# Lapis-Hong/wide_deep

Measured on NVIDIA H100. Metric: CTR examples/sec (train step), higher is better.
Workload: dtype bf16x3 (fp32 operands split into bf16 hi+lo, 3 tensor-core products, fp32 accumulate; 2^-16)

## Files before the change

### include/wd_b200.h

```cpp
#ifndef WD_B200_H_
#define WD_B200_H_

#include <stddef.h>
#include <stdint.h>

#ifdef __cplusplus
extern "C" {
#endif

#define WD_API_VERSION 3

enum { WD_OK = 0, WD_EINVAL = -1, WD_ENODEVICE = -2, WD_ECUDA = -3, WD_ENOMEM = -4, WD_EUNSUPPORTED = -5, WD_ESTATE = -6 };

enum { WD_COL_HASH = 0, WD_COL_VOCAB = 1, WD_COL_IDENTITY = 2, WD_COL_BUCKET = 3, WD_COL_CROSS = 4 };
enum { WD_NORM_NONE = 0, WD_NORM_MINMAX = 1, WD_NORM_STANDARD = 2, WD_NORM_LOG = 3 };
enum { WD_KEY_FIELD = 0, WD_KEY_COLUMN = 1 };
enum { WD_OPT_SGD = 0, WD_OPT_ADAGRAD = 1, WD_OPT_FTRL = 2,
       WD_OPT_ADAM = 3     ,
       WD_OPT_RMSPROP = 4   };
enum { WD_ACT_RELU = 0, WD_ACT_RELU6, WD_ACT_SIGMOID, WD_ACT_TANH, WD_ACT_LEAKY_RELU, WD_ACT_ELU, WD_ACT_SELU,
       WD_ACT_SOFTPLUS, WD_ACT_SOFTSIGN,
       WD_ACT_CRELU    };
enum { WD_MODE_SIMPLE = 0, WD_MODE_FIRST_DENSE, WD_MODE_LAST_DENSE, WD_MODE_DENSE, WD_MODE_RESNET };
enum { WD_GEMM_AUTO = 0, WD_GEMM_FFMA = 1, WD_GEMM_TC3X = 2 ,
// ... 134 lines not shown

int wd_eval_reset(WdModel *m);
int wd_eval_accumulate(WdModel *m, const WdBatch *batch);
int wd_eval_finish(WdModel *m, double *out10);
int wd_eval_accumulate_slot(WdModel *m, int slot);

int wd_fingerprint64_device(const uint8_t *bytes, const int64_t *offsets, int64_t n, uint64_t *out);
uint64_t wd_fingerprint64(const uint8_t *bytes, size_t n);
uint64_t wd_fingerprint_cat64(uint64_t a, uint64_t b);

int wd_debug_column_ids(WdModel *m, int32_t *offsets_out, int64_t offsets_cap, int64_t *ids_out, int64_t ids_cap, int64_t *nnz_out);
int wd_debug_slot(WdModel *m, int slot, int32_t *batch_out, int64_t *nnz_out, int32_t *parts_out, int32_t *offsets_out,
                  uint64_t *keys_out, float *dense_out, float *label_out, float *weight_out);
int wd_debug_deep_input(WdModel *m, float *out, int64_t cap);
int wd_debug_hidden(WdModel *m, int tower, int layer, float *out, int64_t cap);
int64_t wd_launch_count(WdModel *m);
int64_t wd_gemm_fallback_count(WdModel *m);
int wd_graph_stats(WdModel *m, int64_t *out, int32_t n);
int wd_last_timings(WdModel *m, float *ms_out, int cap);
const char *wd_timing_name(WdModel *m, int i);
int wd_set_profile(WdModel *m, int enable);
void *wd_stream(WdModel *m);
int wd_debug_gemm_probe(unsigned long long *out);
void *wd_stream_sparse(WdModel *m, int which);
int wd_sync(WdModel *m);

#define WD_SUMMARY_BUCKETS 1551
enum { WD_SEG_DEEP_INPUT = 0, WD_SEG_HIDDEN = 1, WD_SEG_TOWER_LOGITS = 2, WD_SEG_WIDE_LOGIT = 3 };
int wd_summary_limits(double *out, int32_t cap);
int wd_summary_segments(WdModel *m, int32_t *kind, int32_t *tower, int32_t *layer, int32_t cap);
int wd_summary_arm(WdModel *m);
int wd_summary_read(WdModel *m, int64_t *counts, int64_t *ints, double *reals, int32_t n_segments);

typedef struct WdTsvSpec {
    int32_t n_columns;
    const int32_t *col_role;
    const int32_t *col_target;
    int32_t n_cat_fields, n_dense_fields;
    int32_t multivalue;
    int32_t tf_compat_pad;
    float pos_weight, neg_weight;
    int32_t use_weight;
    int32_t has_label;
} WdTsvSpec;
int64_t wd_tsv_parse(const WdTsvSpec *spec, const char *text, int64_t text_len, int32_t n_lines,
                     int32_t *offsets_out, uint64_t *keys_out, int64_t keys_cap,
// ... 20 lines not shown
```

### wide_deep_b200/_native.py

```python
import ctypes
import os

_HERE = os.path.dirname(os.path.abspath(__file__))
SO_PATH = os.path.join(_HERE, "libwd_b200.so")
_lib = None

OK, EINVAL, ENODEVICE, ECUDA, ENOMEM, EUNSUPPORTED, ESTATE = 0, -1, -2, -3, -4, -5, -6


class NativeError(RuntimeError):
    def __init__(self, code, msg):
        super().__init__("libwd_b200 error %d: %s" % (code, msg))
        self.code = code


class BatchC(ctypes.Structure):
    _fields_ = [("batch_size", ctypes.c_int32), ("cat_offsets", ctypes.c_void_p), ("cat_keys", ctypes.c_void_p),
                ("nnz", ctypes.c_int64), ("dense", ctypes.c_void_p), ("label", ctypes.c_void_p), ("weight", ctypes.c_void_p)]


class TsvSpecC(ctypes.Structure):
    _fields_ = [("n_columns", ctypes.c_int32), ("col_role", ctypes.c_void_p), ("col_target", ctypes.c_void_p),
                ("n_cat_fields", ctypes.c_int32), ("n_dense_fields", ctypes.c_int32), ("multivalue", ctypes.c_int32),
                ("tf_compat_pad", ctypes.c_int32), ("pos_weight", ctypes.c_float), ("neg_weight", ctypes.c_float),
# ... 44 lines not shown
    "wd_shard_eval_accumulate_phase": (ctypes.c_int, [_vp, _i32]),
    "wd_shard_eval_finish": (ctypes.c_int, [_vp, _vp]),
    "wd_eval_reset": (ctypes.c_int, [_vp]),
    "wd_eval_accumulate": (ctypes.c_int, [_vp, _vp]),
    "wd_eval_finish": (ctypes.c_int, [_vp, _vp]),
    "wd_eval_accumulate_slot": (ctypes.c_int, [_vp, ctypes.c_int]),
    "wd_fingerprint64_device": (ctypes.c_int, [_vp, _vp, _i64, _vp]),
    "wd_fingerprint64": (_u64, [ctypes.c_char_p, ctypes.c_size_t]),
    "wd_fingerprint_cat64": (_u64, [_u64, _u64]),
    "wd_debug_column_ids": (ctypes.c_int, [_vp, _vp, _i64, _vp, _i64, ctypes.POINTER(_i64)]),
    "wd_debug_slot": (ctypes.c_int, [_vp, ctypes.c_int, ctypes.POINTER(_i32), ctypes.POINTER(_i64), ctypes.POINTER(_i32), _vp, _vp, _vp,
                                     _vp, _vp]),
    "wd_debug_deep_input": (ctypes.c_int, [_vp, _vp, _i64]),
    "wd_debug_hidden": (ctypes.c_int, [_vp, ctypes.c_int, ctypes.c_int, _vp, _i64]),
    "wd_launch_count": (_i64, [_vp]),
    "wd_gemm_fallback_count": (_i64, [_vp]),
    "wd_graph_stats": (ctypes.c_int, [_vp, ctypes.POINTER(_i64), _i32]),
    "wd_last_timings": (ctypes.c_int, [_vp, _vp, ctypes.c_int]),
    "wd_timing_name": (ctypes.c_char_p, [_vp, ctypes.c_int]),
    "wd_batch_upload_slot": (ctypes.c_int, [_vp, ctypes.c_int, _vp]),
    "wd_batch_prefetch_slot": (ctypes.c_int, [_vp, ctypes.c_int, _vp]),
    "wd_last_loss": (ctypes.c_int, [_vp, _vp]),
    "wd_debug_gemm_probe": (ctypes.c_int, [_vp]),
    "wd_train_step_slot": (ctypes.c_int, [_vp, ctypes.c_int, ctypes.POINTER(ctypes.c_float)]),
    "wd_set_profile": (ctypes.c_int, [_vp, ctypes.c_int]),
    "wd_stream": (_vp, [_vp]),
    "wd_stream_sparse": (_vp, [_vp, ctypes.c_int]),
    "wd_sync": (ctypes.c_int, [_vp]),
    "wd_host_alloc": (ctypes.c_int, [ctypes.c_size_t, ctypes.POINTER(_vp)]),
    "wd_host_free": (ctypes.c_int, [_vp]),
    "wd_tsv_parse": (_i64, [_vp, ctypes.c_char_p, _i64, _i32, _vp, _vp, _i64, _vp, _vp, _vp, _i32]),
    "wd_tsv_index_lines": (_i64, [_vp, _i64, _vp, _vp, _i64]),
    "wd_tsv_parse_lines": (_i64, [_vp, _vp, _vp, _vp, _vp, _i32, _vp, _vp, _i64, _vp, _vp, _vp, _i32]),
    "wd_tsv_gather_lines": (_i64, [_vp, _vp, _vp, _vp, _i32, _vp, _i64, _vp, _i32]),
    "wd_tsv_parse_slot": (ctypes.c_int, [_vp, ctypes.c_int, _vp, _vp, _i64, _vp, _i32]),
    "wd_tsv_parse_stats": (ctypes.c_int, [_vp, ctypes.POINTER(_i64), _i32, _i32]),
    "wd_summary_limits": (ctypes.c_int, [_vp, _i32]),
    "wd_summary_segments": (ctypes.c_int, [_vp, _vp, _vp, _vp, _i32]),
    "wd_summary_arm": (ctypes.c_int, [_vp]),
    "wd_summary_read": (ctypes.c_int, [_vp, _vp, _vp, _vp, _i32]),
}


def lib():
    global _lib
    if _lib is None:
# ... 15 lines not shown
```

### wide_deep_b200/csrc/gemm.cuh

```cuda
#pragma once
#include <cuda.h>
#include <cuda_bf16.h>

#include "common.cuh"

namespace wd {

__device__ __forceinline__ float act_fwd(int kind, float z) {
    switch (kind) {
        case WD_ACT_RELU: return fmaxf(z, 0.f);
        case WD_ACT_RELU6: return fminf(fmaxf(z, 0.f), 6.f);
        case WD_ACT_SIGMOID: return 1.f / (1.f + expf(-z));
        case WD_ACT_TANH: return tanhf(z);
        case WD_ACT_LEAKY_RELU: return z > 0.f ? z : 0.2f * z;
        case WD_ACT_ELU: return z > 0.f ? z : expm1f(z);
        case WD_ACT_SELU: return 1.0507009873554805f * (z > 0.f ? z : 1.6732632423543772f * expm1f(z));
        case WD_ACT_SOFTPLUS: return fmaxf(z, 0.f) + log1pf(expf(-fabsf(z)));
        case WD_ACT_SOFTSIGN: return z / (1.f + fabsf(z));
    }
    return z;
}
__device__ __forceinline__ float act_bwd(int kind, float a) {
    switch (kind) {
        case WD_ACT_RELU: return a > 0.f ? 1.f : 0.f;
// ... 18 lines not shown
    const __nv_bfloat16* lo[kMaxSegs];
};
struct GemmB {
    const float* ptr; int ld;
    const float *tf32_hi, *tf32_lo;
    const __nv_bfloat16 *hi, *lo;
};
enum { EPI_FWD = 0, EPI_STORE = 1, EPI_WGRAD = 2 };
struct Epi {
    float* C; int ldc;
    int accumulate;
    float* A_out; float* H_out; int ldh;
    float* HT; int ldt;
    const float *bias, *gamma, *beta;
    int n_logical, act, bn;
    int m_valid;
    int64_t split_stride;
    __nv_bfloat16 *Hs_hi, *Hs_lo;
    uint64_t reserved[5];
};

int tc_gemm(WdModel* m, int mode, const GemmA& A, const GemmB& B, int M, int N, const Epi& ep, int splits, int ksplit_len);
int tc_gemm_bf16(WdModel* m, int mode, const GemmA& A, const GemmB& B, int M, int N, const Epi& ep, int splits, int ksplit_len);
int make_tensor_map(CUtensorMap* map, CUtensorMapDataType dtype, const void* ptr, int rows, int cols, int ld, int box_rows);

struct DropArgs { float rate; unsigned long long seed; const unsigned int* step; int layer_id; unsigned int row0; };
__device__ __forceinline__ unsigned long long splitmix64_dev(unsigned long long x) {
    x += 0x9E3779B97F4A7C15ULL;
    x = (x ^ (x >> 30)) * 0xBF58476D1CE4E5B9ULL;
    x = (x ^ (x >> 27)) * 0x94D049BB133111EBULL;
    return x ^ (x >> 31);
}
__device__ __forceinline__ unsigned long long drop_key(const DropArgs& d) {
    return splitmix64_dev(d.seed ^ ((unsigned long long)(*d.step) * 0x9E3779B97F4A7C15ULL) ^ ((unsigned long long)d.layer_id << 48));
}
__device__ __forceinline__ float drop_mult(unsigned long long key, unsigned int m, unsigned int n, float rate, float inv_keep) {
    const unsigned long long r = splitmix64_dev(key ^ ((unsigned long long)m * 65536ULL + n));
    const float u = (float)(unsigned int)(r >> 40) * (1.f / 16777216.f);
    return u >= rate ? inv_keep : 0.f;
}

__device__ __forceinline__ float bn_out(float a, const float* __restrict__ gamma, const float* __restrict__ beta, int n, int bn) {
    return bn ? fmaf(a, gamma[n] * 0.99950037468777f, beta[n]) : a;
}

__device__ __forceinline__ void split_bf16(float x, __nv_bfloat16& hi, __nv_bfloat16& lo) {
    hi = __float2bfloat16_rn(x);
// ... 18 lines not shown
```

### wide_deep_b200/csrc/gemm_bf16.cu

```cuda
#include <cuda.h>
#include <stdlib.h>

#include <algorithm>
#include <type_traits>

#include "common.cuh"
#include "gemm.cuh"
#include "wgmma_ptx.cuh"

namespace wd {

namespace {

constexpr int QBM = 128;
constexpr int QBN = 128;
constexpr int QNST = 3;
constexpr int QBK = 64;
constexpr int Q_THREADS = 384;

struct QMaps {
    CUtensorMap a_hi[kMaxSegs], a_lo[kMaxSegs];
    CUtensorMap b_hi, b_lo;
};
struct QSegs { int n; int k[kMaxSegs]; int koff[kMaxSegs]; };

__device__ unsigned long long g_probe[32 * 8];
__device__ __forceinline__ unsigned long long gtime() { unsigned long long t; asm volatile("mov.u64 %0, %globaltimer;" : "=l"(t)); return t; }
#define PROBE(i) do { if (probe >= 0 && blockIdx.x == 0 && (threadIdx.x & 127) == 0) g_probe[probe * 8 + (i)] = gtime(); } while (0)

template <int MODE>
__global__ void __launch_bounds__(Q_THREADS, 1) tc_gemm_bf16_kernel(const __grid_constant__ QMaps maps, const QSegs segs, int M, int N, int ktot,
                                                                   int ksplit_len, int nsplit, Epi ep, int probe) {
    extern __shared__ uint8_t smem_raw[];
    uint8_t* base = reinterpret_cast<uint8_t*>((reinterpret_cast<uintptr_t>(smem_raw) + 1023) & ~uintptr_t(1023));
    constexpr bool A_MN = MODE == EPI_WGRAD;
    constexpr bool B_MN = MODE == EPI_FWD || MODE == EPI_WGRAD;
    constexpr int A_BYTES = QBM * 128, B_BYTES = QBN * 128;
    constexpr int STAGE_BYTES = 2 * (A_BYTES + B_BYTES);
    auto a_hi = [&](int s) { return base + s * STAGE_BYTES; };
    auto a_lo = [&](int s) { return base + s * STAGE_BYTES + A_BYTES; };
    auto b_hi = [&](int s) { return base + s * STAGE_BYTES + 2 * A_BYTES; };
    auto b_lo = [&](int s) { return base + s * STAGE_BYTES + 2 * A_BYTES + B_BYTES; };
    uint64_t* bars = reinterpret_cast<uint64_t*>(base + QNST * STAGE_BYTES);
    uint64_t* full = bars; uint64_t* empty = bars + QNST;
    float* epi_vec = reinterpret_cast<float*>(base + QNST * STAGE_BYTES + 64);

    const int warp = threadIdx.x >> 5, lane = threadIdx.x & 31, wg = threadIdx.x >> 7;
    const int tiles_n = (N + QBN - 1) / QBN, tiles_m = (M + QBM - 1) / QBM;
    const int ntiles = tiles_n * tiles_m * nsplit;
    int nkb_all = 0;
    for (int s = 0; s < segs.n; ++s) nkb_all += (segs.k[s] + QBK - 1) / QBK;
    auto tile_range = [&](int tile, int& m0, int& n0, int& z, int& kbeg, int& nkb) {
        z = tile / (tiles_n * tiles_m);
        int r = tile % (tiles_n * tiles_m);
        m0 = (r / tiles_n) * QBM;
        n0 = (r % tiles_n) * QBN;
        kbeg = 0;
        nkb = nkb_all;
        if (MODE == EPI_WGRAD) {
            kbeg = z * ksplit_len;
            int kend = min(ktot, kbeg + ksplit_len);
            nkb = kend > kbeg ? (kend - kbeg + QBK - 1) / QBK : 0;
        }
    };

    if (threadIdx.x == 0) {
        for (int s = 0; s < QNST; ++s) { mbar_init(&full[s], 1); mbar_init(&empty[s], 8); }
        asm volatile("fence.mbarrier_init.release.cluster;" ::: "memory");
    }
    __syncthreads();

    if (wg == 0) {
        reg_dealloc<40>();
        PROBE(0);
        if (warp == 0 && lane == 0) {
            int g = 0;
            for (int tile = blockIdx.x; tile < ntiles; tile += gridDim.x) {
                int m0, n0, z, kbeg, nkb;
                tile_range(tile, m0, n0, z, kbeg, nkb);
                int seg = 0, kin = 0;
                for (int kb = 0; kb < nkb; ++kb, ++g) {
                    const int s = g % QNST, it = g / QNST;
                    if (it > 0) mbar_wait(&empty[s], (it - 1) & 1);
                    int ka, kbcoord;
                    if (MODE == EPI_WGRAD) { ka = kbeg + kb * QBK; kbcoord = ka; }
                    else {
                        if (kin >= segs.k[seg]) { ++seg; kin = 0; }
                        ka = kin; kbcoord = segs.koff[seg] + kin;
                        kin += QBK;
                    }
                    mbar_expect_tx(&full[s], 2 * (A_BYTES + B_BYTES));
                    if (!A_MN) {
                        tma_load_2d(a_hi(s), &maps.a_hi[seg], &full[s], ka, m0);
                        tma_load_2d(a_lo(s), &maps.a_lo[seg], &full[s], ka, m0);
                    } else {
#pragma unroll
                        for (int i = 0; i < QBM / 64; ++i) {
                            tma_load_2d(a_hi(s) + i * 8192, &maps.a_hi[seg], &full[s], m0 + 64 * i, ka);
                            tma_load_2d(a_lo(s) + i * 8192, &maps.a_lo[seg], &full[s], m0 + 64 * i, ka);
                        }
                    }
                    if (!B_MN) {
                        tma_load_2d(b_hi(s), &maps.b_hi, &full[s], kbcoord, n0);
                        tma_load_2d(b_lo(s), &maps.b_lo, &full[s], kbcoord, n0);
                    } else {
#pragma unroll
                        for (int i = 0; i < QBN / 64; ++i) {
                            tma_load_2d(b_hi(s) + i * 8192, &maps.b_hi, &full[s], n0 + 64 * i, kbcoord);
                            tma_load_2d(b_lo(s) + i * 8192, &maps.b_lo, &full[s], n0 + 64 * i, kbcoord);
                        }
                    }
                }
            }
        }
    } else {
        reg_alloc<232>();
        const int cw = wg - 1, cwarp = warp - 4;
        constexpr uint32_t a_step = A_MN ? 2048u : 32u, b_step = B_MN ? 2048u : 32u;
        constexpr int TA = A_MN ? 1 : 0, TB = B_MN ? 1 : 0;
        float d[QBN / 2];
        int g = 0, use = 0;
        for (int tile = blockIdx.x; tile < ntiles; tile += gridDim.x) {
            int m0, n0, z, kbeg, nkb;
            tile_range(tile, m0, n0, z, kbeg, nkb);
            if (nkb == 0) {
#pragma unroll
                for (int i = 0; i < QBN / 2; ++i) d[i] = 0.f;
            }
            const int ct = threadIdx.x - 128;
            float pre[2] = {0.f, 0.f};
            if (MODE == EPI_FWD) {
#pragma unroll
                for (int i = 0; i < 2; ++i) {
                    const int v = ct + 256 * i, c = n0 + (v & 127);
                    const bool in = c < ep.n_logical;
                    if (v < 128) pre[i] = in ? __ldg(ep.bias + c) : 0.f;
                    else if (v < 256) pre[i] = (in && ep.bn) ? __ldg(ep.gamma + c) * 0.99950037468777f : 1.f;
                    else if (v < 384) pre[i] = (in && ep.bn) ? __ldg(ep.beta + c) : 0.f;
                }
            }
            int prev = -1;
            for (int kb = 0; kb < nkb; ++kb, ++g) {
                const int s = g % QNST, it = g / QNST;
                mbar_wait(&full[s], it & 1);
                if (g == 0) PROBE(1);
                const uint32_t sa_hi = smem_u32(a_hi(s)) + cw * 8192, sa_lo = smem_u32(a_lo(s)) + cw * 8192;
                const uint32_t sb_hi = smem_u32(b_hi(s)), sb_lo = smem_u32(b_lo(s));
                wgmma_fence();
#pragma unroll
                for (int k = 0; k < QBK / 16; ++k) {
                    const uint64_t da_hi = A_MN ? make_desc_mn(sa_hi + k * a_step) : make_desc(sa_hi + k * a_step);
                    const uint64_t da_lo = A_MN ? make_desc_mn(sa_lo + k * a_step) : make_desc(sa_lo + k * a_step);
                    const uint64_t db_hi = B_MN ? make_desc_mn(sb_hi + k * b_step) : make_desc(sb_hi + k * b_step);
                    const uint64_t db_lo = B_MN ? make_desc_mn(sb_lo + k * b_step) : make_desc(sb_lo + k * b_step);
                    wgmma_bf16<TA, TB>(d, da_lo, db_hi, (kb > 0 || k > 0) ? 1u : 0u);
                    wgmma_bf16<TA, TB>(d, da_hi, db_lo, 1u);
                    wgmma_bf16<TA, TB>(d, da_hi, db_hi, 1u);
                }
                wgmma_commit();
                if (prev >= 0) {
                    wgmma_wait<1>();
                    if (lane == 0) mbar_arrive(&empty[prev]);
                }
                prev = s;
            }
            wgmma_wait<0>();
            if (prev >= 0 && lane == 0) mbar_arrive(&empty[prev]);
            if (cwarp == 0) PROBE(use == 0 ? 2 : 3);
            const float* ev = epi_vec + (use & 1) * 384;
            if (MODE == EPI_FWD) {
                epi_vec[(use & 1) * 384 + ct] = pre[0];
                if (ct < 128) epi_vec[(use & 1) * 384 + ct + 256] = pre[1];
                bar_sync(1, 256);
            }

            const int r0 = m0 + cw * 64 + (warp & 3) * 16 + (lane >> 2);
            const int cq = 2 * (lane & 3);
            auto epilogue = [&](auto relu) {
                constexpr bool RELU = decltype(relu)::value;
                uint32_t qh[2][2] = {}, ql[2][2] = {};
#pragma unroll
                for (int j = 0; j < QBN / 8; ++j) {
                    const int c = n0 + 8 * j + cq;
                    if (n0 + 8 * j < N) {
                        if (MODE == EPI_FWD) {
                            const bool in0 = c < ep.n_logical, in1 = c + 1 < ep.n_logical;
                            const int cl = 8 * j + cq;
                            const float b0 = ev[cl], b1 = ev[cl + 1], g0 = ev[128 + cl], g1 = ev[129 + cl], e0 = ev[256 + cl], e1 = ev[257 + cl];
#pragma unroll
                            for (int hh = 0; hh < 2; ++hh) {
                                const int r = r0 + 8 * hh;
                                if (r >= M) continue;
                                const bool rv = r < ep.m_valid;
                                float a0 = 0.f, a1 = 0.f, h0 = 0.f, h1 = 0.f;
                                if (rv && in0) { a0 = RELU ? fmaxf(d[4 * j + 2 * hh] + b0, 0.f) : act_fwd(ep.act, d[4 * j + 2 * hh] + b0); h0 = fmaf(a0, g0, e0); }
                                if (rv && in1) { a1 = RELU ? fmaxf(d[4 * j + 2 * hh + 1] + b1, 0.f) : act_fwd(ep.act, d[4 * j + 2 * hh + 1] + b1); h1 = fmaf(a1, g1, e1); }
                                const int64_t o = (int64_t)r * ep.ldh + c;
                                if (ep.A_out != ep.H_out) *reinterpret_cast<float2*>(ep.A_out + o) = make_float2(a0, a1);
                                if (ep.H_out) *reinterpret_cast<float2*>(ep.H_out + o) = make_float2(h0, h1);
                                split_pair(h0, h1, qh[j & 1][hh], ql[j & 1][hh]);
                            }
// ... 11 lines not shown
                                    vl.x = q < 2 ? l0a : l1a; vl.y = q < 2 ? l0b : l1b;
                                    const int r = r0 + 8 * hh;
                                    if (r >= M) continue;
                                    const int64_t o = (int64_t)r * ep.ldh + cp;
                                    *reinterpret_cast<uint2*>(ep.Hs_hi + o) = vh;
                                    *reinterpret_cast<uint2*>(ep.Hs_lo + o) = vl;
                                }
                            }
                        } else {
                            float* Cb = ep.C + (MODE == EPI_WGRAD ? (int64_t)z * ep.split_stride : 0);
#pragma unroll
                            for (int hh = 0; hh < 2; ++hh) {
                                const int r = r0 + 8 * hh;
                                if (r >= M) continue;
                                float2* pc = reinterpret_cast<float2*>(Cb + (int64_t)r * ep.ldc + c);
                                float2 o = make_float2(d[4 * j + 2 * hh], d[4 * j + 2 * hh + 1]);
                                if (MODE == EPI_STORE && ep.accumulate) { const float2 p = *pc; o.x += p.x; o.y += p.y; }
                                *pc = o;
                            }
                        }
                    }
                }
            };
            if (MODE == EPI_FWD && ep.act == WD_ACT_RELU) epilogue(std::true_type{});
            else epilogue(std::false_type{});
            if (cwarp == 0) PROBE(use == 0 ? 4 : 5);
            ++use;
        }
    }
}

int g_probe_slot = 0;

template <int MODE>
int launch_q(WdModel* m, const QMaps& maps, const QSegs& segs, int M, int N, int ktot, int splits, int ksplit_len, const Epi& ep) {
    constexpr int smem = QNST * 2 * (QBM * 128 + QBN * 128) + 1024 + 64 + 2 * 384 * 4;
    static bool configured = false;
    static int num_sms = 0;
    if (!configured) {
        WD_CUDA(cudaFuncSetAttribute(tc_gemm_bf16_kernel<MODE>, cudaFuncAttributeMaxDynamicSharedMemorySize, smem));
        WD_CUDA(cudaDeviceGetAttribute(&num_sms, cudaDevAttrMultiProcessorCount, m->device));
        configured = true;
    }
    const int nsplit = MODE == EPI_WGRAD ? splits : 1;
    const int ntiles = ((N + QBN - 1) / QBN) * ((M + QBM - 1) / QBM) * nsplit;
    static const bool probe_on = getenv("WD_GEMM_PROBE") != nullptr;
    const int probe = probe_on ? (g_probe_slot++ & 31) : -1;
    tc_gemm_bf16_kernel<MODE><<<ntiles < num_sms ? ntiles : num_sms, Q_THREADS, smem, m->stream>>>(maps, segs, M, N, ktot, ksplit_len, nsplit, ep, probe);
    m->launches++;
    WD_CUDA(cudaGetLastError());
    return WD_OK;
}

}

extern "C" int wd_debug_gemm_probe(unsigned long long* out) {
    cudaDeviceSynchronize();
    cudaError_t e = cudaMemcpyFromSymbol(out, g_probe, sizeof(unsigned long long) * 32 * 8);
    g_probe_slot = 0;
    return e == cudaSuccess ? 0 : -1;
}

int tc_gemm_bf16(WdModel* m, int mode, const GemmA& A, const GemmB& B, int M, int N, const Epi& ep, int splits, int ksplit_len) {
    constexpr CUtensorMapDataType BF16 = CU_TENSOR_MAP_DATA_TYPE_BFLOAT16;
    if (N % 32 != 0 || A.n > kMaxSegs || !B.hi || !B.lo) { set_error("bf16 GEMM engine: unsupported operands"); return WD_EUNSUPPORTED; }
    QMaps maps;
    QSegs segs{};
    segs.n = A.n;
    int rc, ktot = 0;
    const bool a_mn = mode == EPI_WGRAD, b_mn = mode == EPI_FWD || mode == EPI_WGRAD;
    for (int s = 0; s < A.n; ++s) {
        if (!A.hi[s] || !A.lo[s]) { set_error("bf16 GEMM engine: operand without hi/lo copies"); return WD_EINVAL; }
        if (!a_mn) {
            if ((rc = make_tensor_map(&maps.a_hi[s], BF16, A.hi[s], M, A.k[s], A.ld[s], QBM))) return rc;
            if ((rc = make_tensor_map(&maps.a_lo[s], BF16, A.lo[s], M, A.k[s], A.ld[s], QBM))) return rc;
        } else {
            if ((rc = make_tensor_map(&maps.a_hi[s], BF16, A.hi[s], A.k[s], M, A.ld[s], 64))) return rc;
            if ((rc = make_tensor_map(&maps.a_lo[s], BF16, A.lo[s], A.k[s], M, A.ld[s], 64))) return rc;
        }
        segs.k[s] = A.k[s]; segs.koff[s] = ktot;
        ktot += A.k[s];
    }
    for (int s = A.n; s < kMaxSegs; ++s) { maps.a_hi[s] = maps.a_hi[0]; maps.a_lo[s] = maps.a_lo[0]; }
    if (!b_mn) {
        if ((rc = make_tensor_map(&maps.b_hi, BF16, B.hi, N, ktot, B.ld, QBN))) return rc;
        if ((rc = make_tensor_map(&maps.b_lo, BF16, B.lo, N, ktot, B.ld, QBN))) return rc;
    } else {
        if ((rc = make_tensor_map(&maps.b_hi, BF16, B.hi, ktot, N, B.ld, 64))) return rc;
        if ((rc = make_tensor_map(&maps.b_lo, BF16, B.lo, ktot, N, B.ld, 64))) return rc;
    }
    if (mode == EPI_WGRAD) ksplit_len = (ksplit_len + QBK - 1) / QBK * QBK;
    if (mode == EPI_FWD && (!ep.Hs_hi || !ep.Hs_lo)) { set_error("bf16 GEMM engine: epilogue without hi/lo outputs"); return WD_EINVAL; }
    if (mode == EPI_FWD) return launch_q<EPI_FWD>(m, maps, segs, M, N, ktot, splits, ksplit_len, ep);
    if (mode == EPI_STORE) return launch_q<EPI_STORE>(m, maps, segs, M, N, ktot, splits, ksplit_len, ep);
    return launch_q<EPI_WGRAD>(m, maps, segs, M, N, ktot, splits, ksplit_len, ep);
}

}
```

### wide_deep_b200/csrc/gemm_tc.cu

```cuda
#include <cuda.h>
#include <stdlib.h>

#include <mutex>
#include <unordered_map>

#include "common.cuh"
#include "gemm.cuh"
#include "wgmma_ptx.cuh"

namespace wd {

constexpr int TBM = 128;
constexpr int TBN = 128;
constexpr int TBK = 32;
constexpr int TSTAGES = 3;
constexpr int TC_THREADS = 512;

struct TcMaps {
    CUtensorMap a[kMaxSegs];
    CUtensorMap b;
    CUtensorMap b_lo;
};

template <int MODE, bool SPLIT3>
// ... 174 lines not shown
                    }
                }
            }
        }
    }
}

typedef CUresult (*EncodeFn)(CUtensorMap*, CUtensorMapDataType, cuuint32_t, void*, const cuuint64_t*, const cuuint64_t*,
                             const cuuint32_t*, const cuuint32_t*, CUtensorMapInterleave, CUtensorMapSwizzle,
                             CUtensorMapL2promotion, CUtensorMapFloatOOBfill);
static EncodeFn g_encode = nullptr;

static int get_encode() {
    if (g_encode) return WD_OK;
    void* fn = nullptr;
    cudaDriverEntryPointQueryResult qres;
    cudaError_t e = cudaGetDriverEntryPoint("cuTensorMapEncodeTiled", &fn, cudaEnableDefault, &qres);
    if (e != cudaSuccess || !fn) { set_error("cuTensorMapEncodeTiled unavailable: %s", cudaGetErrorString(e)); return WD_ECUDA; }
    g_encode = (EncodeFn)fn;
    return WD_OK;
}

struct MapKey {
    const void* p; int rows, cols, ld, box_rows, esize;
    bool operator==(const MapKey& o) const { return p == o.p && rows == o.rows && cols == o.cols && ld == o.ld && box_rows == o.box_rows && esize == o.esize; }
};
struct MapKeyHash {
    size_t operator()(const MapKey& k) const {
        uint64_t h = (uint64_t)(uintptr_t)k.p * 0x9E3779B97F4A7C15ull;
        h ^= ((uint64_t)(uint32_t)k.rows << 32 | (uint32_t)k.cols) * 0xC2B2AE3D27D4EB4Full;
        h ^= ((uint64_t)(uint32_t)k.ld << 20 | (uint64_t)(uint32_t)k.box_rows << 4 | (uint32_t)k.esize) * 0x165667B19E3779F9ull;
        return (size_t)(h ^ (h >> 29));
    }
};
static std::unordered_map<MapKey, CUtensorMap, MapKeyHash> g_map_cache;
static std::mutex g_map_mutex;
static bool map_cache_get(const MapKey& k, CUtensorMap* out) {
    std::lock_guard<std::mutex> lock(g_map_mutex);
    auto it = g_map_cache.find(k);
    if (it == g_map_cache.end()) return false;
    *out = it->second;
    return true;
}
static void map_cache_put(const MapKey& k, const CUtensorMap& v) {
    std::lock_guard<std::mutex> lock(g_map_mutex);
    if (g_map_cache.size() > 4096) g_map_cache.clear();
    g_map_cache[k] = v;
}
void tc_map_cache_clear() {
    std::lock_guard<std::mutex> lock(g_map_mutex);
    g_map_cache.clear();
}

int make_tensor_map(CUtensorMap* map, CUtensorMapDataType dtype, const void* ptr, int rows, int cols, int ld, int box_rows) {
    int rc = get_encode();
    if (rc) return rc;
    const int esize = dtype == CU_TENSOR_MAP_DATA_TYPE_FLOAT32 ? 4 : 2;
    const MapKey key{ptr, rows, cols, ld, box_rows, esize};
    if (map_cache_get(key, map)) return WD_OK;
    cuuint64_t dims[2] = {(cuuint64_t)cols, (cuuint64_t)rows};
    cuuint64_t strides[1] = {(cuuint64_t)ld * esize};
    cuuint32_t box[2] = {(cuuint32_t)(128 / esize), (cuuint32_t)box_rows};
    cuuint32_t estr[2] = {1, 1};
    CUresult r = g_encode(map, dtype, 2, const_cast<void*>(ptr), dims, strides, box, estr, CU_TENSOR_MAP_INTERLEAVE_NONE,
                          CU_TENSOR_MAP_SWIZZLE_128B, CU_TENSOR_MAP_L2_PROMOTION_L2_256B, CU_TENSOR_MAP_FLOAT_OOB_FILL_NONE);
    if (r != CUDA_SUCCESS) {
        set_error("cuTensorMapEncodeTiled failed (%d) rows=%d cols=%d ld=%d element=%d bytes", (int)r, rows, cols, ld, esize);
        return WD_ECUDA;
    }
    map_cache_put(key, *map);
    return WD_OK;
}

template <int MODE, bool SPLIT3>
static int launch_tc(WdModel* m, const TcMaps& maps, int nseg, const int* segk, int M, int N, int ktot, int splits, int ksplit_len, const Epi& ep) {
    constexpr int A_BYTES = TBM * 128, B_BYTES = TBN * 128;
    constexpr int NST = TSTAGES;
    constexpr int smem = NST * (SPLIT3 ? 2 : 1) * (A_BYTES + B_BYTES) + 1024 + 128;
    int4 s01 = make_int4(segk[0], segk[1], segk[2], segk[3]), s23 = make_int4(segk[4], segk[5], segk[6], segk[7]);
    static bool configured = false;
    static int num_sms = 0;
    if (!configured) {
        WD_CUDA(cudaFuncSetAttribute(tc_gemm_kernel<MODE, SPLIT3>, cudaFuncAttributeMaxDynamicSharedMemorySize, smem));
        WD_CUDA(cudaDeviceGetAttribute(&num_sms, cudaDevAttrMultiProcessorCount, m->device));
        configured = true;
    }
    const int nsplit = MODE == EPI_WGRAD ? splits : 1;
    const int ntiles = ((N + TBN - 1) / TBN) * ((M + TBM - 1) / TBM) * nsplit;
// ... 38 lines not shown
```

### wide_deep_b200/csrc/wgmma_ptx.cuh

```cuda
#pragma once
#include <cuda.h>
#include <stdint.h>

namespace wd {

__device__ __forceinline__ uint32_t smem_u32(const void* p) { return (uint32_t)__cvta_generic_to_shared(p); }
__device__ __forceinline__ void mbar_init(uint64_t* bar, uint32_t count) {
    asm volatile("mbarrier.init.shared::cta.b64 [%0], %1;" ::"r"(smem_u32(bar)), "r"(count));
}
__device__ __forceinline__ void mbar_expect_tx(uint64_t* bar, uint32_t bytes) {
    asm volatile("mbarrier.arrive.expect_tx.shared::cta.b64 _, [%0], %1;" ::"r"(smem_u32(bar)), "r"(bytes) : "memory");
}
__device__ __forceinline__ void mbar_arrive(uint64_t* bar) {
    asm volatile("mbarrier.arrive.shared::cta.b64 _, [%0];" ::"r"(smem_u32(bar)) : "memory");
}
__device__ __forceinline__ void mbar_wait(uint64_t* bar, uint32_t parity) {
    asm volatile(
        "{\n\t.reg .pred p;\n\t"
        "WAIT_LOOP:\n\t"
        "mbarrier.try_wait.parity.shared::cta.b64 p, [%0], %1;\n\t"
        "@p bra WAIT_DONE;\n\t"
        "bra WAIT_LOOP;\n\t"
        "WAIT_DONE:\n\t}" ::"r"(smem_u32(bar)), "r"(parity) : "memory");
}
__device__ __forceinline__ void tma_load_2d(void* dst, const CUtensorMap* map, uint64_t* bar, int c0, int c1) {
    asm volatile("cp.async.bulk.tensor.2d.shared::cluster.global.mbarrier::complete_tx::bytes [%0], [%1, {%3, %4}], [%2];"
                 ::"r"(smem_u32(dst)), "l"(reinterpret_cast<uint64_t>(map)), "r"(smem_u32(bar)), "r"(c0), "r"(c1) : "memory");
}

__device__ __forceinline__ void bar_sync(int id, int n) { asm volatile("bar.sync %0, %1;" ::"r"(id), "r"(n) : "memory"); }

template <int N> __device__ __forceinline__ void reg_dealloc() { asm volatile("setmaxnreg.dec.sync.aligned.u32 %0;" ::"n"(N)); }
template <int N> __device__ __forceinline__ void reg_alloc() { asm volatile("setmaxnreg.inc.sync.aligned.u32 %0;" ::"n"(N)); }

__device__ __forceinline__ void wgmma_fence() { asm volatile("wgmma.fence.sync.aligned;" ::: "memory"); }
__device__ __forceinline__ void wgmma_commit() { asm volatile("wgmma.commit_group.sync.aligned;" ::: "memory"); }
template <int N> __device__ __forceinline__ void wgmma_wait() { asm volatile("wgmma.wait_group.sync.aligned %0;" ::"n"(N) : "memory"); }

__device__ __forceinline__ uint64_t make_desc(uint32_t saddr) {
    uint64_t d = 0;
    d |= (uint64_t)((saddr >> 4) & 0x3FFF);
    d |= (uint64_t)1 << 16;
    d |= (uint64_t)(1024 >> 4) << 32;
    d |= (uint64_t)1 << 62;
    return d;
}

__device__ __forceinline__ uint64_t make_desc_mn(uint32_t saddr) {
    uint64_t d = 0;
    d |= (uint64_t)((saddr >> 4) & 0x3FFF);
    d |= (uint64_t)(8192 >> 4) << 16;
    d |= (uint64_t)(1024 >> 4) << 32;
    d |= (uint64_t)1 << 62;
    return d;
}

template <int TA, int TB>
__device__ __forceinline__ void wgmma_bf16(float (&d)[64], uint64_t desc_a, uint64_t desc_b, uint32_t accumulate) {
    asm volatile(
        "{\n\t.reg .pred p;\n\tsetp.ne.b32 p, %66, 0;\n\t"
        "wgmma.mma_async.sync.aligned.m64n128k16.f32.bf16.bf16 {"
        "%0, %1, %2, %3, %4, %5, %6, %7, %8, %9, %10, %11, %12, %13, %14, %15, %16, %17, %18, %19, %20, %21, %22, %23, %24, %25, "
        "%26, %27, %28, %29, %30, %31, %32, %33, %34, %35, %36, %37, %38, %39, %40, %41, %42, %43, %44, %45, %46, %47, %48, %49, "
        "%50, %51, %52, %53, %54, %55, %56, %57, %58, %59, %60, %61, %62, %63}, "
        "%64, %65, p, 1, 1, %67, %68;\n\t}"
        : "+f"(d[0]), "+f"(d[1]), "+f"(d[2]), "+f"(d[3]), "+f"(d[4]), "+f"(d[5]), "+f"(d[6]), "+f"(d[7]),
          "+f"(d[8]), "+f"(d[9]), "+f"(d[10]), "+f"(d[11]), "+f"(d[12]), "+f"(d[13]), "+f"(d[14]), "+f"(d[15]),
          "+f"(d[16]), "+f"(d[17]), "+f"(d[18]), "+f"(d[19]), "+f"(d[20]), "+f"(d[21]), "+f"(d[22]), "+f"(d[23]),
          "+f"(d[24]), "+f"(d[25]), "+f"(d[26]), "+f"(d[27]), "+f"(d[28]), "+f"(d[29]), "+f"(d[30]), "+f"(d[31]),
          "+f"(d[32]), "+f"(d[33]), "+f"(d[34]), "+f"(d[35]), "+f"(d[36]), "+f"(d[37]), "+f"(d[38]), "+f"(d[39]),
          "+f"(d[40]), "+f"(d[41]), "+f"(d[42]), "+f"(d[43]), "+f"(d[44]), "+f"(d[45]), "+f"(d[46]), "+f"(d[47]),
          "+f"(d[48]), "+f"(d[49]), "+f"(d[50]), "+f"(d[51]), "+f"(d[52]), "+f"(d[53]), "+f"(d[54]), "+f"(d[55]),
          "+f"(d[56]), "+f"(d[57]), "+f"(d[58]), "+f"(d[59]), "+f"(d[60]), "+f"(d[61]), "+f"(d[62]), "+f"(d[63])
        : "l"(desc_a), "l"(desc_b), "r"(accumulate), "n"(TA), "n"(TB));
// ... 22 lines not shown
```

Before: 10.48 million.

## Add 256-row BF16x3 GEMM tiles with 64B swizzle and deeper pipeline

Halves the K block to 32 with 64-byte swizzled TMA boxes and matching wgmma descriptors, which allows more pipeline stages (6 or 4). It also adds a 256-row M tile for the data-gradient GEMM, chosen by a wave-count heuristic when K is large, so each B tile is reused across two 64-row halves per warpgroup. The intent is better operand reuse and latency hiding. The cost is more register pressure, twice as many barrier waits per K, and K padding to 64 that relies on TMA out-of-bounds zero fill.

```diff
diff --git a/include/wd_b200.h b/include/wd_b200.h
--- a/include/wd_b200.h
+++ b/include/wd_b200.h
@@ -180,6 +180,7 @@
 int wd_set_profile(WdModel *m, int enable);
 void *wd_stream(WdModel *m);
 int wd_debug_gemm_probe(unsigned long long *out);
+int wd_debug_gemm_tile_rows(int rows);
 void *wd_stream_sparse(WdModel *m, int which);
 int wd_sync(WdModel *m);
 
diff --git a/wide_deep_b200/_native.py b/wide_deep_b200/_native.py
--- a/wide_deep_b200/_native.py
+++ b/wide_deep_b200/_native.py
@@ -90,6 +90,7 @@
     "wd_batch_prefetch_slot": (ctypes.c_int, [_vp, ctypes.c_int, _vp]),
     "wd_last_loss": (ctypes.c_int, [_vp, _vp]),
     "wd_debug_gemm_probe": (ctypes.c_int, [_vp]),
+    "wd_debug_gemm_tile_rows": (ctypes.c_int, [ctypes.c_int]),
     "wd_train_step_slot": (ctypes.c_int, [_vp, ctypes.c_int, ctypes.POINTER(ctypes.c_float)]),
     "wd_set_profile": (ctypes.c_int, [_vp, ctypes.c_int]),
     "wd_stream": (_vp, [_vp]),
diff --git a/wide_deep_b200/csrc/gemm.cuh b/wide_deep_b200/csrc/gemm.cuh
--- a/wide_deep_b200/csrc/gemm.cuh
+++ b/wide_deep_b200/csrc/gemm.cuh
@@ -64,7 +64,7 @@
 
 int tc_gemm(WdModel* m, int mode, const GemmA& A, const GemmB& B, int M, int N, const Epi& ep, int splits, int ksplit_len);
 int tc_gemm_bf16(WdModel* m, int mode, const GemmA& A, const GemmB& B, int M, int N, const Epi& ep, int splits, int ksplit_len);
-int make_tensor_map(CUtensorMap* map, CUtensorMapDataType dtype, const void* ptr, int rows, int cols, int ld, int box_rows);
+int make_tensor_map(CUtensorMap* map, CUtensorMapDataType dtype, const void* ptr, int rows, int cols, int ld, int box_rows, int box_bytes = 128);
 
 struct DropArgs { float rate; unsigned long long seed; const unsigned int* step; int layer_id; unsigned int row0; };
 __device__ __forceinline__ unsigned long long splitmix64_dev(unsigned long long x) {
diff --git a/wide_deep_b200/csrc/gemm_bf16.cu b/wide_deep_b200/csrc/gemm_bf16.cu
--- a/wide_deep_b200/csrc/gemm_bf16.cu
+++ b/wide_deep_b200/csrc/gemm_bf16.cu
@@ -12,11 +12,13 @@
 
 namespace {
 
-constexpr int QBM = 128;
 constexpr int QBN = 128;
-constexpr int QNST = 3;
-constexpr int QBK = 64;
+constexpr int QBK = 32;
+constexpr int QKP = 64;
 constexpr int Q_THREADS = 384;
+
+template <int BM> constexpr int q_stages() { return BM == 128 ? 6 : 4; }
+template <int BM> constexpr int q_smem_bytes() { return q_stages<BM>() * 2 * (BM + QBN) * QBK * 2 + 1024 + 128 + 2 * 384 * 4; }
 
 struct QMaps {
     CUtensorMap a_hi[kMaxSegs], a_lo[kMaxSegs];
@@ -28,14 +30,19 @@
 __device__ __forceinline__ unsigned long long gtime() { unsigned long long t; asm volatile("mov.u64 %0, %globaltimer;" : "=l"(t)); return t; }
 #define PROBE(i) do { if (probe >= 0 && blockIdx.x == 0 && (threadIdx.x & 127) == 0) g_probe[probe * 8 + (i)] = gtime(); } while (0)
 
-template <int MODE>
+template <int MODE, int QBM>
 __global__ void __launch_bounds__(Q_THREADS, 1) tc_gemm_bf16_kernel(const __grid_constant__ QMaps maps, const QSegs segs, int M, int N, int ktot,
                                                                    int ksplit_len, int nsplit, Epi ep, int probe) {
     extern __shared__ uint8_t smem_raw[];
     uint8_t* base = reinterpret_cast<uint8_t*>((reinterpret_cast<uintptr_t>(smem_raw) + 1023) & ~uintptr_t(1023));
     constexpr bool A_MN = MODE == EPI_WGRAD;
     constexpr bool B_MN = MODE == EPI_FWD || MODE == EPI_WGRAD;
-    constexpr int A_BYTES = QBM * 128, B_BYTES = QBN * 128;
+    constexpr int QNST = q_stages<QBM>();
+    constexpr int MH = QBM / 128;
+    constexpr int ROW_BYTES = QBK * 2;
+    constexpr int MN_BOX = 64 * ROW_BYTES;
+    static_assert(QBM == 128 || MODE == EPI_STORE, "256-row tiles run the data gradient only (both operands K-major)");
+    constexpr int A_BYTES = QBM * ROW_BYTES, B_BYTES = QBN * ROW_BYTES;
     constexpr int STAGE_BYTES = 2 * (A_BYTES + B_BYTES);
     auto a_hi = [&](int s) { return base + s * STAGE_BYTES; };
     auto a_lo = [&](int s) { return base + s * STAGE_BYTES + A_BYTES; };
@@ -43,13 +50,14 @@
     auto b_lo = [&](int s) { return base + s * STAGE_BYTES + 2 * A_BYTES + B_BYTES; };
     uint64_t* bars = reinterpret_cast<uint64_t*>(base + QNST * STAGE_BYTES);
     uint64_t* full = bars; uint64_t* empty = bars + QNST;
-    float* epi_vec = reinterpret_cast<float*>(base + QNST * STAGE_BYTES + 64);
+    static_assert(2 * QNST * 8 <= 128, "mbarriers overlap the epilogue constants");
+    float* epi_vec = reinterpret_cast<float*>(base + QNST * STAGE_BYTES + 128);
 
     const int warp = threadIdx.x >> 5, lane = threadIdx.x & 31, wg = threadIdx.x >> 7;
     const int tiles_n = (N + QBN - 1) / QBN, tiles_m = (M + QBM - 1) / QBM;
     const int ntiles = tiles_n * tiles_m * nsplit;
     int nkb_all = 0;
-    for (int s = 0; s < segs.n; ++s) nkb_all += (segs.k[s] + QBK - 1) / QBK;
+    for (int s = 0; s < segs.n; ++s) nkb_all += (segs.k[s] + QKP - 1) / QKP * (QKP / QBK);
     auto tile_range = [&](int tile, int& m0, int& n0, int& z, int& kbeg, int& nkb) {
         z = tile / (tiles_n * tiles_m);
         int r = tile % (tiles_n * tiles_m);
@@ -60,7 +68,7 @@
         if (MODE == EPI_WGRAD) {
             kbeg = z * ksplit_len;
             int kend = min(ktot, kbeg + ksplit_len);
-            nkb = kend > kbeg ? (kend - kbeg + QBK - 1) / QBK : 0;
+            nkb = kend > kbeg ? (kend - kbeg + QKP - 1) / QKP * (QKP / QBK) : 0;
         }
     };
 
@@ -85,7 +93,7 @@
                     int ka, kbcoord;
                     if (MODE == EPI_WGRAD) { ka = kbeg + kb * QBK; kbcoord = ka; }
                     else {
-                        if (kin >= segs.k[seg]) { ++seg; kin = 0; }
+                        if (kin >= (segs.k[seg] + QKP - 1) / QKP * QKP) { ++seg; kin = 0; }
                         ka = kin; kbcoord = segs.koff[seg] + kin;
                         kin += QBK;
                     }
@@ -96,8 +104,8 @@
                     } else {
 #pragma unroll
                         for (int i = 0; i < QBM / 64; ++i) {
-                            tma_load_2d(a_hi(s) + i * 8192, &maps.a_hi[seg], &full[s], m0 + 64 * i, ka);
-                            tma_load_2d(a_lo(s) + i * 8192, &maps.a_lo[seg], &full[s], m0 + 64 * i, ka);
+                            tma_load_2d(a_hi(s) + i * MN_BOX, &maps.a_hi[seg], &full[s], m0 + 64 * i, ka);
+                            tma_load_2d(a_lo(s) + i * MN_BOX, &maps.a_lo[seg], &full[s], m0 + 64 * i, ka);
                         }
                     }
                     if (!B_MN) {
@@ -106,8 +114,8 @@
                     } else {
 #pragma unroll
                         for (int i = 0; i < QBN / 64; ++i) {
-                            tma_load_2d(b_hi(s) + i * 8192, &maps.b_hi, &full[s], n0 + 64 * i, kbcoord);
-                            tma_load_2d(b_lo(s) + i * 8192, &maps.b_lo, &full[s], n0 + 64 * i, kbcoord);
+                            tma_load_2d(b_hi(s) + i * MN_BOX, &maps.b_hi, &full[s], n0 + 64 * i, kbcoord);
+                            tma_load_2d(b_lo(s) + i * MN_BOX, &maps.b_lo, &full[s], n0 + 64 * i, kbcoord);
                         }
                     }
                 }
@@ -118,14 +126,16 @@
         const int cw = wg - 1, cwarp = warp - 4;
         constexpr uint32_t a_step = A_MN ? 2048u : 32u, b_step = B_MN ? 2048u : 32u;
         constexpr int TA = A_MN ? 1 : 0, TB = B_MN ? 1 : 0;
-        float d[QBN / 2];
+        float d[MH][QBN / 2];
         int g = 0, use = 0;
         for (int tile = blockIdx.x; tile < ntiles; tile += gridDim.x) {
             int m0, n0, z, kbeg, nkb;
             tile_range(tile, m0, n0, z, kbeg, nkb);
             if (nkb == 0) {
 #pragma unroll
-                for (int i = 0; i < QBN / 2; ++i) d[i] = 0.f;
+                for (int h = 0; h < MH; ++h)
+#pragma unroll
+                    for (int i = 0; i < QBN / 2; ++i) d[h][i] = 0.f;
             }
             const int ct = threadIdx.x - 128;
             float pre[2] = {0.f, 0.f};
@@ -144,18 +154,22 @@
                 const int s = g % QNST, it = g / QNST;
                 mbar_wait(&full[s], it & 1);
                 if (g == 0) PROBE(1);
-                const uint32_t sa_hi = smem_u32(a_hi(s)) + cw * 8192, sa_lo = smem_u32(a_lo(s)) + cw * 8192;
+                const uint32_t sa_hi = smem_u32(a_hi(s)) + cw * (QBM / 2) * ROW_BYTES, sa_lo = smem_u32(a_lo(s)) + cw * (QBM / 2) * ROW_BYTES;
                 const uint32_t sb_hi = smem_u32(b_hi(s)), sb_lo = smem_u32(b_lo(s));
                 wgmma_fence();
 #pragma unroll
                 for (int k = 0; k < QBK / 16; ++k) {
-                    const uint64_t da_hi = A_MN ? make_desc_mn(sa_hi + k * a_step) : make_desc(sa_hi + k * a_step);
-                    const uint64_t da_lo = A_MN ? make_desc_mn(sa_lo + k * a_step) : make_desc(sa_lo + k * a_step);
-                    const uint64_t db_hi = B_MN ? make_desc_mn(sb_hi + k * b_step) : make_desc(sb_hi + k * b_step);
-                    const uint64_t db_lo = B_MN ? make_desc_mn(sb_lo + k * b_step) : make_desc(sb_lo + k * b_step);
-                    wgmma_bf16<TA, TB>(d, da_lo, db_hi, (kb > 0 || k > 0) ? 1u : 0u);
-                    wgmma_bf16<TA, TB>(d, da_hi, db_lo, 1u);
-                    wgmma_bf16<TA, TB>(d, da_hi, db_hi, 1u);
+#pragma unroll
+                    for (int h = 0; h < MH; ++h) {
+                        const uint32_t ah = sa_hi + h * 64 * ROW_BYTES + k * a_step, al = sa_lo + h * 64 * ROW_BYTES + k * a_step;
+                        const uint64_t da_hi = A_MN ? make_desc_mn(ah, MN_BOX) : make_desc_sw64(ah);
+                        const uint64_t da_lo = A_MN ? make_desc_mn(al, MN_BOX) : make_desc_sw64(al);
+                        const uint64_t db_hi = B_MN ? make_desc_mn(sb_hi + k * b_step, MN_BOX) : make_desc_sw64(sb_hi + k * b_step);
+                        const uint64_t db_lo = B_MN ? make_desc_mn(sb_lo + k * b_step, MN_BOX) : make_desc_sw64(sb_lo + k * b_step);
+                        wgmma_bf16<TA, TB>(d[h], da_lo, db_hi, (kb > 0 || k > 0) ? 1u : 0u);
+                        wgmma_bf16<TA, TB>(d[h], da_hi, db_lo, 1u);
+                        wgmma_bf16<TA, TB>(d[h], da_hi, db_hi, 1u);
+                    }
                 }
                 wgmma_commit();
                 if (prev >= 0) {
@@ -174,9 +188,8 @@
                 bar_sync(1, 256);
             }
 
-            const int r0 = m0 + cw * 64 + (warp & 3) * 16 + (lane >> 2);
             const int cq = 2 * (lane & 3);
-            auto epilogue = [&](auto relu) {
+            auto epilogue = [&](auto relu, const float (&d)[QBN / 2], const int r0) {
                 constexpr bool RELU = decltype(relu)::value;
                 uint32_t qh[2][2] = {}, ql[2][2] = {};
 #pragma unroll
@@ -234,8 +247,12 @@
                     }
                 }
             };
-            if (MODE == EPI_FWD && ep.act == WD_ACT_RELU) epilogue(std::true_type{});
-            else epilogue(std::false_type{});
+#pragma unroll
+            for (int h = 0; h < MH; ++h) {
+                const int r0 = m0 + cw * (QBM / 2) + h * 64 + (warp & 3) * 16 + (lane >> 2);
+                if (MODE == EPI_FWD && ep.act == WD_ACT_RELU) epilogue(std::true_type{}, d[h], r0);
+                else epilogue(std::false_type{}, d[h], r0);
+            }
             if (cwarp == 0) PROBE(use == 0 ? 4 : 5);
             ++use;
         }
@@ -244,24 +261,32 @@
 
 int g_probe_slot = 0;
 
-template <int MODE>
-int launch_q(WdModel* m, const QMaps& maps, const QSegs& segs, int M, int N, int ktot, int splits, int ksplit_len, const Epi& ep) {
-    constexpr int smem = QNST * 2 * (QBM * 128 + QBN * 128) + 1024 + 64 + 2 * 384 * 4;
+template <int MODE, int QBM>
+int launch_q(WdModel* m, const QMaps& maps, const QSegs& segs, int M, int N, int ktot, int splits, int ksplit_len, const Epi& ep, int num_sms) {
+    constexpr int smem = q_smem_bytes<QBM>();
     static bool configured = false;
-    static int num_sms = 0;
     if (!configured) {
-        WD_CUDA(cudaFuncSetAttribute(tc_gemm_bf16_kernel<MODE>, cudaFuncAttributeMaxDynamicSharedMemorySize, smem));
-        WD_CUDA(cudaDeviceGetAttribute(&num_sms, cudaDevAttrMultiProcessorCount, m->device));
+        WD_CUDA(cudaFuncSetAttribute(tc_gemm_bf16_kernel<MODE, QBM>, cudaFuncAttributeMaxDynamicSharedMemorySize, smem));
         configured = true;
     }
     const int nsplit = MODE == EPI_WGRAD ? splits : 1;
     const int ntiles = ((N + QBN - 1) / QBN) * ((M + QBM - 1) / QBM) * nsplit;
     static const bool probe_on = getenv("WD_GEMM_PROBE") != nullptr;
     const int probe = probe_on ? (g_probe_slot++ & 31) : -1;
-    tc_gemm_bf16_kernel<MODE><<<ntiles < num_sms ? ntiles : num_sms, Q_THREADS, smem, m->stream>>>(maps, segs, M, N, ktot, ksplit_len, nsplit, ep, probe);
+    tc_gemm_bf16_kernel<MODE, QBM><<<ntiles < num_sms ? ntiles : num_sms, Q_THREADS, smem, m->stream>>>(maps, segs, M, N, ktot, ksplit_len, nsplit, ep, probe);
     m->launches++;
     WD_CUDA(cudaGetLastError());
     return WD_OK;
+}
+
+int g_tile_rows = 0;
+
+int q_tile_rows(int mode, int M, int N, int K, int num_sms) {
+    if (mode != EPI_STORE || g_tile_rows == 128) return 128;
+    if (g_tile_rows == 256) return 256;
+    const int tn = (N + QBN - 1) / QBN;
+    const int waves128 = ((M + 127) / 128 * tn + num_sms - 1) / num_sms, waves256 = ((M + 255) / 256 * tn + num_sms - 1) / num_sms;
+    return K >= 512 && 2 * waves256 <= waves128 ? 256 : 128;
 }
 
 }
@@ -273,39 +298,50 @@
     return e == cudaSuccess ? 0 : -1;
 }
 
+extern "C" int wd_debug_gemm_tile_rows(int rows) {
+    if (rows != 0 && rows != 128 && rows != 256) return -1;
+    g_tile_rows = rows;
+    return 0;
+}
+
 int tc_gemm_bf16(WdModel* m, int mode, const GemmA& A, const GemmB& B, int M, int N, const Epi& ep, int splits, int ksplit_len) {
     constexpr CUtensorMapDataType BF16 = CU_TENSOR_MAP_DATA_TYPE_BFLOAT16;
     if (N % 32 != 0 || A.n > kMaxSegs || !B.hi || !B.lo) { set_error("bf16 GEMM engine: unsupported operands"); return WD_EUNSUPPORTED; }
+    static int num_sms = 0;
+    if (!num_sms) WD_CUDA(cudaDeviceGetAttribute(&num_sms, cudaDevAttrMultiProcessorCount, m->device));
     QMaps maps;
     QSegs segs{};
     segs.n = A.n;
-    int rc, ktot = 0;
+    int rc, ktot = 0, kall = 0;
+    for (int s = 0; s < A.n; ++s) kall += A.k[s];
+    const int bm = q_tile_rows(mode, M, N, kall, num_sms);
     const bool a_mn = mode == EPI_WGRAD, b_mn = mode == EPI_FWD || mode == EPI_WGRAD;
     for (int s = 0; s < A.n; ++s) {
         if (!A.hi[s] || !A.lo[s]) { set_error("bf16 GEMM engine: operand without hi/lo copies"); return WD_EINVAL; }
         if (!a_mn) {
-            if ((rc = make_tensor_map(&maps.a_hi[s], BF16, A.hi[s], M, A.k[s], A.ld[s], QBM))) return rc;
-            if ((rc = make_tensor_map(&maps.a_lo[s], BF16, A.lo[s], M, A.k[s], A.ld[s], QBM))) return rc;
+            if ((rc = make_tensor_map(&maps.a_hi[s], BF16, A.hi[s], M, A.k[s], A.ld[s], bm, 2 * QBK))) return rc;
+            if ((rc = make_tensor_map(&maps.a_lo[s], BF16, A.lo[s], M, A.k[s], A.ld[s], bm, 2 * QBK))) return rc;
         } else {
-            if ((rc = make_tensor_map(&maps.a_hi[s], BF16, A.hi[s], A.k[s], M, A.ld[s], 64))) return rc;
-            if ((rc = make_tensor_map(&maps.a_lo[s], BF16, A.lo[s], A.k[s], M, A.ld[s], 64))) return rc;
+            if ((rc = make_tensor_map(&maps.a_hi[s], BF16, A.hi[s], A.k[s], M, A.ld[s], QBK))) return rc;
+            if ((rc = make_tensor_map(&maps.a_lo[s], BF16, A.lo[s], A.k[s], M, A.ld[s], QBK))) return rc;
         }
         segs.k[s] = A.k[s]; segs.koff[s] = ktot;
         ktot += A.k[s];
     }
     for (int s = A.n; s < kMaxSegs; ++s) { maps.a_hi[s] = maps.a_hi[0]; maps.a_lo[s] = maps.a_lo[0]; }
     if (!b_mn) {
-        if ((rc = make_tensor_map(&maps.b_hi, BF16, B.hi, N, ktot, B.ld, QBN))) return rc;
-        if ((rc = make_tensor_map(&maps.b_lo, BF16, B.lo, N, ktot, B.ld, QBN))) return rc;
+        if ((rc = make_tensor_map(&maps.b_hi, BF16, B.hi, N, ktot, B.ld, QBN, 2 * QBK))) return rc;
+        if ((rc = make_tensor_map(&maps.b_lo, BF16, B.lo, N, ktot, B.ld, QBN, 2 * QBK))) return rc;
     } else {
-        if ((rc = make_tensor_map(&maps.b_hi, BF16, B.hi, ktot, N, B.ld, 64))) return rc;
-        if ((rc = make_tensor_map(&maps.b_lo, BF16, B.lo, ktot, N, B.ld, 64))) return rc;
-    }
-    if (mode == EPI_WGRAD) ksplit_len = (ksplit_len + QBK - 1) / QBK * QBK;
+        if ((rc = make_tensor_map(&maps.b_hi, BF16, B.hi, ktot, N, B.ld, QBK))) return rc;
+        if ((rc = make_tensor_map(&maps.b_lo, BF16, B.lo, ktot, N, B.ld, QBK))) return rc;
+    }
+    if (mode == EPI_WGRAD) ksplit_len = (ksplit_len + QKP - 1) / QKP * QKP;
     if (mode == EPI_FWD && (!ep.Hs_hi || !ep.Hs_lo)) { set_error("bf16 GEMM engine: epilogue without hi/lo outputs"); return WD_EINVAL; }
-    if (mode == EPI_FWD) return launch_q<EPI_FWD>(m, maps, segs, M, N, ktot, splits, ksplit_len, ep);
-    if (mode == EPI_STORE) return launch_q<EPI_STORE>(m, maps, segs, M, N, ktot, splits, ksplit_len, ep);
-    return launch_q<EPI_WGRAD>(m, maps, segs, M, N, ktot, splits, ksplit_len, ep);
-}
-
-}
+    if (mode == EPI_FWD) return launch_q<EPI_FWD, 128>(m, maps, segs, M, N, ktot, splits, ksplit_len, ep, num_sms);
+    if (mode == EPI_STORE) return bm == 256 ? launch_q<EPI_STORE, 256>(m, maps, segs, M, N, ktot, splits, ksplit_len, ep, num_sms)
+                                            : launch_q<EPI_STORE, 128>(m, maps, segs, M, N, ktot, splits, ksplit_len, ep, num_sms);
+    return launch_q<EPI_WGRAD, 128>(m, maps, segs, M, N, ktot, splits, ksplit_len, ep, num_sms);
+}
+
+}
diff --git a/wide_deep_b200/csrc/gemm_tc.cu b/wide_deep_b200/csrc/gemm_tc.cu
--- a/wide_deep_b200/csrc/gemm_tc.cu
+++ b/wide_deep_b200/csrc/gemm_tc.cu
@@ -220,14 +220,17 @@
 }
 
 struct MapKey {
-    const void* p; int rows, cols, ld, box_rows, esize;
-    bool operator==(const MapKey& o) const { return p == o.p && rows == o.rows && cols == o.cols && ld == o.ld && box_rows == o.box_rows && esize == o.esize; }
+    const void* p; int rows, cols, ld, box_rows, esize, box_bytes;
+    bool operator==(const MapKey& o) const {
+        return p == o.p && rows == o.rows && cols == o.cols && ld == o.ld && box_rows == o.box_rows && esize == o.esize && box_bytes == o.box_bytes;
+    }
 };
 struct MapKeyHash {
     size_t operator()(const MapKey& k) const {
         uint64_t h = (uint64_t)(uintptr_t)k.p * 0x9E3779B97F4A7C15ull;
         h ^= ((uint64_t)(uint32_t)k.rows << 32 | (uint32_t)k.cols) * 0xC2B2AE3D27D4EB4Full;
         h ^= ((uint64_t)(uint32_t)k.ld << 20 | (uint64_t)(uint32_t)k.box_rows << 4 | (uint32_t)k.esize) * 0x165667B19E3779F9ull;
+        h ^= (uint64_t)k.box_bytes;
         return (size_t)(h ^ (h >> 29));
     }
 };
@@ -250,18 +253,18 @@
     g_map_cache.clear();
 }
 
-int make_tensor_map(CUtensorMap* map, CUtensorMapDataType dtype, const void* ptr, int rows, int cols, int ld, int box_rows) {
+int make_tensor_map(CUtensorMap* map, CUtensorMapDataType dtype, const void* ptr, int rows, int cols, int ld, int box_rows, int box_bytes) {
     int rc = get_encode();
     if (rc) return rc;
     const int esize = dtype == CU_TENSOR_MAP_DATA_TYPE_FLOAT32 ? 4 : 2;
-    const MapKey key{ptr, rows, cols, ld, box_rows, esize};
+    const MapKey key{ptr, rows, cols, ld, box_rows, esize, box_bytes};
     if (map_cache_get(key, map)) return WD_OK;
     cuuint64_t dims[2] = {(cuuint64_t)cols, (cuuint64_t)rows};
     cuuint64_t strides[1] = {(cuuint64_t)ld * esize};
-    cuuint32_t box[2] = {(cuuint32_t)(128 / esize), (cuuint32_t)box_rows};
+    cuuint32_t box[2] = {(cuuint32_t)(box_bytes / esize), (cuuint32_t)box_rows};
     cuuint32_t estr[2] = {1, 1};
     CUresult r = g_encode(map, dtype, 2, const_cast<void*>(ptr), dims, strides, box, estr, CU_TENSOR_MAP_INTERLEAVE_NONE,
-                          CU_TENSOR_MAP_SWIZZLE_128B, CU_TENSOR_MAP_L2_PROMOTION_L2_256B, CU_TENSOR_MAP_FLOAT_OOB_FILL_NONE);
+                          box_bytes == 128 ? CU_TENSOR_MAP_SWIZZLE_128B : CU_TENSOR_MAP_SWIZZLE_64B, CU_TENSOR_MAP_L2_PROMOTION_L2_256B, CU_TENSOR_MAP_FLOAT_OOB_FILL_NONE);
     if (r != CUDA_SUCCESS) {
         set_error("cuTensorMapEncodeTiled failed (%d) rows=%d cols=%d ld=%d element=%d bytes", (int)r, rows, cols, ld, esize);
         return WD_ECUDA;
diff --git a/wide_deep_b200/csrc/wgmma_ptx.cuh b/wide_deep_b200/csrc/wgmma_ptx.cuh
--- a/wide_deep_b200/csrc/wgmma_ptx.cuh
+++ b/wide_deep_b200/csrc/wgmma_ptx.cuh
@@ -46,10 +46,19 @@
     return d;
 }
 
-__device__ __forceinline__ uint64_t make_desc_mn(uint32_t saddr) {
+__device__ __forceinline__ uint64_t make_desc_sw64(uint32_t saddr) {
     uint64_t d = 0;
     d |= (uint64_t)((saddr >> 4) & 0x3FFF);
-    d |= (uint64_t)(8192 >> 4) << 16;
+    d |= (uint64_t)1 << 16;
+    d |= (uint64_t)(512 >> 4) << 32;
+    d |= (uint64_t)2 << 62;
+    return d;
+}
+
+__device__ __forceinline__ uint64_t make_desc_mn(uint32_t saddr, uint32_t lbo) {
+    uint64_t d = 0;
+    d |= (uint64_t)((saddr >> 4) & 0x3FFF);
+    d |= (uint64_t)((lbo >> 4) & 0x3FFF) << 16;
     d |= (uint64_t)(1024 >> 4) << 32;
     d |= (uint64_t)1 << 62;
     return d;
```

After: 10.53 million, median of 6. No clear change (+0.4%).
